# TimD1/vcfdist

Hardware: AMD Instinct MI355X
Metric: supercluster-alignments/sec (higher is better)
Workload: dtype int32; 1 GPU; wgs_synth; superclusters_per_gpu=1000000, span_dist=lognormal(median 20, sigma 1.2) clip [4,10000]

## Files before the change

include/vcfdist_pr.h:

```cpp
#ifndef VCFDIST_PR_H_
#define VCFDIST_PR_H_

#include <stddef.h>
#include <stdint.h>

#ifdef __cplusplus
extern "C" {
#endif

#define VPR_HAPS 4
#define VPR_ALNS 4

#define VPR_PTR_VARIANT 1
#define VPR_PTR_VAR_BEG 2
#define VPR_PTR_VAR_END 4
#define VPR_PTR_INS_LOC 8

#define VPR_TYPE_SUB 1
#define VPR_TYPE_INS 2
#define VPR_TYPE_DEL 3

#define VPR_ERRTYPE_TP 0
#define VPR_ERRTYPE_FP 1
#define VPR_ERRTYPE_FN 2
// ... 42 lines not shown

typedef struct vpr_variants {
    int32_t n_sc;
    int32_t n_ctg;
    const int64_t *ctg_off;
    const uint8_t *ctg_seq;
    const int32_t *sc_ctg;
    const int32_t *sc_beg;
    const int32_t *sc_end;
    const int64_t *var_off[VPR_HAPS];
    const int32_t *var_pos[VPR_HAPS];
    const uint8_t *var_type[VPR_HAPS];
    const float   *var_qual[VPR_HAPS];
    const int64_t *var_ref_off[VPR_HAPS];
    const int32_t *var_ref_len[VPR_HAPS];
    const int64_t *var_alt_off[VPR_HAPS];
    const int32_t *var_alt_len[VPR_HAPS];
    const uint8_t *allele_pool[VPR_HAPS];
} vpr_variants;

typedef struct vpr_config {
    int32_t device;
    float   max_qual;
    double  credit_threshold;
    double  phase_threshold;
    int64_t workspace_bytes;
    int32_t band_mode;
    int32_t flags;
} vpr_config;
#define VPR_CFG_DENSE_S16 1
#define VPR_CFG_TIE_SMALL_LOGS 2
#define VPR_CFG_GUARD_ALLOC 4
#define VPR_CFG_HAP_DEDUP 16
#define VPR_CFG_KEEP_PATHS 8

typedef struct vpr_results {
    int32_t  *aln_dist;
    uint8_t  *aln_end_plane;
    uint8_t  *aln_beg_plane;
    uint32_t *aln_status;
    int32_t  *sc_phase;
    int32_t  *orig_phase_dist;
    int32_t  *swap_phase_dist;
    uint8_t  *errtype[VPR_HAPS][2];
    int32_t  *sync_group[VPR_HAPS][2];
    float    *credit[VPR_HAPS][2];
    int32_t  *ref_ed[VPR_HAPS][2];
    int32_t  *query_ed[VPR_HAPS][2];
    float    *callq[VPR_HAPS][2];
} vpr_results;

typedef struct vpr_timing {
    double ms_total;
    double ms_prep;
    double ms_fwd;
    double ms_bwd;
    double ms_walk;
    double ms_ed;
    int64_t n_fwd_launches;
    int64_t cells_dense;
    int64_t cells_touched;
    int64_t bytes_algorithmic;
    int64_t n_band_retries;
    int64_t n_tie_replays;
    double  ms_tie;
    double  ms_wall;
// ... 114 lines not shown
```

vcfdist_amd/_abi.py:

```python
import ctypes as C

import numpy as np

HAPS = 4
ALNS = 4

PTR_VARIANT, PTR_VAR_BEG, PTR_VAR_END, PTR_INS_LOC = 1, 2, 4, 8
TYPE_SUB, TYPE_INS, TYPE_DEL = 1, 2, 3
ERRTYPE_TP, ERRTYPE_FP, ERRTYPE_FN, ERRTYPE_UN = 0, 1, 2, 5
PHASE_ORIG, PHASE_SWAP, PHASE_NONE = 0, 1, 2
PLANE_QUERY, PLANE_REF = 0, 1

ST_SWAP_TIE = 1
ST_WARN_REF_ED = 2
ST_WARN_QUERY_ED = 4
ST_WARN_EXCEEDS = 8
ST_WARN_ZERO_ED = 16
ST_ERR_NO_PTR = 32
ST_ERR_UNFINISHED = 64
ST_ERR_LIMIT = 128
ST_WARN_MASK = ST_WARN_REF_ED | ST_WARN_QUERY_ED | ST_WARN_EXCEEDS | ST_WARN_ZERO_ED

P_i64 = C.POINTER(C.c_int64)
P_i32 = C.POINTER(C.c_int32)
# ... 18 lines not shown
    _fields_ = [
        ("n_sc", C.c_int32), ("n_ctg", C.c_int32),
        ("ctg_off", P_i64), ("ctg_seq", P_u8),
        ("sc_ctg", P_i32), ("sc_beg", P_i32), ("sc_end", P_i32),
        ("var_off", P_i64 * HAPS), ("var_pos", P_i32 * HAPS), ("var_type", P_u8 * HAPS),
        ("var_qual", P_f32 * HAPS), ("var_ref_off", P_i64 * HAPS), ("var_ref_len", P_i32 * HAPS),
        ("var_alt_off", P_i64 * HAPS), ("var_alt_len", P_i32 * HAPS),
        ("allele_pool", P_u8 * HAPS),
    ]


class VprConfig(C.Structure):
    _fields_ = [
        ("device", C.c_int32), ("max_qual", C.c_float),
        ("credit_threshold", C.c_double), ("phase_threshold", C.c_double),
        ("workspace_bytes", C.c_int64), ("band_mode", C.c_int32), ("flags", C.c_int32),
    ]


class VprResults(C.Structure):
    _fields_ = [
        ("aln_dist", P_i32), ("aln_end_plane", P_u8), ("aln_beg_plane", P_u8), ("aln_status", P_u32),
        ("sc_phase", P_i32), ("orig_phase_dist", P_i32), ("swap_phase_dist", P_i32),
        ("errtype", (P_u8 * 2) * HAPS), ("sync_group", (P_i32 * 2) * HAPS),
        ("credit", (P_f32 * 2) * HAPS), ("ref_ed", (P_i32 * 2) * HAPS),
        ("query_ed", (P_i32 * 2) * HAPS), ("callq", (P_f32 * 2) * HAPS),
    ]


CFG_DENSE_S16 = 1
CFG_TIE_SMALL_LOGS = 2
CFG_GUARD_ALLOC = 4
CFG_KEEP_PATHS = 8
CFG_HAP_DEDUP = 16


class VprTiming(C.Structure):
    _fields_ = [
        ("ms_total", C.c_double), ("ms_prep", C.c_double), ("ms_fwd", C.c_double),
        ("ms_bwd", C.c_double), ("ms_walk", C.c_double), ("ms_ed", C.c_double),
        ("n_fwd_launches", C.c_int64), ("cells_dense", C.c_int64), ("cells_touched", C.c_int64),
        ("bytes_algorithmic", C.c_int64), ("n_band_retries", C.c_int64),
        ("n_tie_replays", C.c_int64), ("ms_tie", C.c_double),
        ("ms_wall", C.c_double), ("ms_wall_phase", C.c_double * 6), ("ms_host_alloc", C.c_double),
        ("ms_host_blocked", C.c_double), ("n_alignments_computed", C.c_int64), ("n_device_allocs", C.c_int64), ("n_device_frees", C.c_int64),
        ("n_host_allocs", C.c_int64), ("n_lane1_seen", C.c_int64), ("n_lane1_finished", C.c_int64), ("n_lane1_waves_dropped", C.c_int64),
    ]


class VprLaunchStat(C.Structure):
    _fields_ = [
        ("kind", C.c_int32), ("threads", C.c_int32), ("cells_per_thread", C.c_int32), ("n_units", C.c_int32),
        ("cells", C.c_int64), ("bytes_algorithmic", C.c_int64), ("ms", C.c_double),
        ("cells_dense", C.c_int64), ("kernel", C.c_char * 32),
    ]


class VprSynthParams(C.Structure):
    _fields_ = [
        ("seed", C.c_uint64), ("n_sc", C.c_int32), ("len_mode", C.c_int32),
        ("len_a", C.c_double), ("len_b", C.c_double),
        ("len_min", C.c_int32), ("len_max", C.c_int32),
        ("p_repeat", C.c_double), ("var_per_base", C.c_double), ("p_snp", C.c_double),
        ("indel_mean", C.c_double), ("p_hom", C.c_double), ("p_keep", C.c_double),
        ("p_drop", C.c_double), ("max_qual", C.c_int32), ("reserved", C.c_int32),
        ("p_sv", C.c_double), ("sv_min", C.c_int32), ("sv_max", C.c_int32),
# ... 462 lines not shown
```

vcfdist_amd/csrc/pr_api.hip:

```cpp
#include <hip/hip_runtime.h>
#include <hip/hip_ext.h>
#include <dlfcn.h>

#include <algorithm>
#include <atomic>
#include <chrono>
#include <cstdarg>
#include <cstdio>
#include <cstdlib>
#include <cstring>
#include <condition_variable>
#include <deque>
#include <functional>
#include <mutex>
#include <string>
#include <thread>
#include <tuple>
#include <unordered_map>
#include <unordered_set>
#include <vector>

#include "../../include/vcfdist_pr.h"
#include "pr_device.h"
#include "pr_plan.h"
// ... 61 lines not shown
}
__global__ void __launch_bounds__(64) k_zl_hdr(BatchOffsets O, const int32_t *__restrict__ order, int n_short, ZlWave *__restrict__ hdr) {
    const int w = blockIdx.x, lane = threadIdx.x;
    const int j = w * 64 + lane;
    int lq = 0, lr = 0, lt = 0;
    if (j < n_short) {
        const int a = order[j];
        const int sc = a >> 2, i = a & 3, qs = i >> 1, ts = 2 + (i & 1);
        lq = int32_t(O.hap_off[qs][sc + 1] - O.hap_off[qs][sc]);
        lt = int32_t(O.hap_off[ts][sc + 1] - O.hap_off[ts][sc]);
        lr = int32_t(O.ref_off[sc + 1] - O.ref_off[sc]);
    }
#pragma unroll
    for (int o = 32; o; o >>= 1) {
        lq = max(lq, __shfl_xor(lq, o)); lr = max(lr, __shfl_xor(lr, o)); lt = max(lt, __shfl_xor(lt, o));
    }
    if (lane == 0) {
        ZlWave W;
        W.in_off = 0; W.log_off = 0; W.mq = lq; W.mr = lr; W.mt = lt; W.pad = 0;
        hdr[w] = W;
    }
}
__global__ void __launch_bounds__(1024) k_zl_scan(ZlWave *__restrict__ hdr, int n_waves, int64_t *__restrict__ totals) {
    __shared__ int64_t s_in[1024], s_log[1024];
    __shared__ int s_len;
    const int tid = threadIdx.x;
    if (tid == 0) s_len = 0;
    const int per = (n_waves + 1023) / 1024;
    const int b = min(n_waves, tid * per), e = min(n_waves, b + per);
    int64_t si = 0, sl = 0;
    int lm = 0;
    for (int k = b; k < e; k++) {
        const ZlWave W = hdr[k];
        si += 64 * (int64_t(W.mq) + W.mr + W.mt); sl += 80 * int64_t(W.mt);
        lm = max(lm, max(W.mq, max(W.mr, W.mt)));
    }
    s_in[tid] = si; s_log[tid] = sl;
    __syncthreads();
    for (int o = 1; o < 1024; o <<= 1) {
        const int64_t ai = tid >= o ? s_in[tid - o] : 0, al = tid >= o ? s_log[tid - o] : 0;
        __syncthreads();
        s_in[tid] += ai; s_log[tid] += al;
        __syncthreads();
    }
    int64_t oi = s_in[tid] - si, ol = s_log[tid] - sl;
    for (int k = b; k < e; k++) {
        ZlWave W = hdr[k];
        W.in_off = oi; W.log_off = ol;
        oi += 64 * (int64_t(W.mq) + W.mr + W.mt); ol += 80 * int64_t(W.mt);
        hdr[k] = W;
    }
    if (lm) atomicMax(&s_len, lm);
    __syncthreads();
    if (tid == 1023) { totals[0] = s_in[1023]; totals[1] = s_log[1023]; totals[2] = s_len; }
}


int class_of(int len) {
    for (int k = 0; k < N_CLASSES; k++)
        if (len <= CLASSES[k].max_len) return k;
    return -1;
}

size_t fwd_lds_bytes(int cls, int Lq, int Lr) {
    const int C = CLASSES[cls].c, NT = CLASSES[cls].nt;
    const size_t PQ = (Lq + C - 1) / C * C, PR = (Lr + C - 1) / C * C;
    return (PQ + PR + 8 + 2 * (NT / 64)) * 4;
}
size_t bwd_lds_bytes(int cls, int Lq, int Lr, bool s16 = false) {
    const int C = CLASSES[cls].c, NT = CLASSES[cls].nt;
    const size_t PQ = (Lq + C - 1) / C * C, PR = (Lr + C - 1) / C * C;
    const size_t FQ = (PQ + 16 + 15) & ~size_t(15), FR = (PR + 16 + 15) & ~size_t(15);
    return (((PQ + PR + 8) * (s16 ? 2 : 4) + 15) & ~size_t(15)) + 2 * (FQ + FR) + 4 * (NT / 64) * 4 + 16;
}
bool s16_ok(const AlnDesc &d) { return d.qv_end - d.qv_beg < 32000; }

bool dense_fits(const AlnDesc &d) {
    const int cls = class_of(std::max(d.Lq, d.Lr));
    if (cls < 0 || cls >= STRIP_ONLY_CLS) return false;
    return fwd_lds_bytes(cls, d.Lq, d.Lr) <= LDS_MAX &&
           (bwd_lds_bytes(cls, d.Lq, d.Lr) <= LDS_MAX || (s16_ok(d) && bwd_lds_bytes(cls, d.Lq, d.Lr, true) <= LDS_MAX));
}
// ... 538 lines not shown
int prep_zero_lane(vpr_handle *h) {
    const Plan &P = h->plan0;
    std::vector<ZlWave> &hdr = h->zl_hdr_host;
    hdr.clear();
    h->zl_wave0.assign(P.chunks.size(), 0);
    int64_t in_words = 0, log_max = 0, in_chunk_max = 0, n_short_max = 0;
    int32_t len_max = 0;
    for (size_t ci = 0; ci < P.chunks.size(); ci++) {
        const Chunk &ch = P.chunks[ci];
        h->zl_wave0[ci] = int64_t(hdr.size());
        const int64_t first = ch.work_off + ch.n_long, n_short = ch.count - ch.n_long;
        const int64_t in_words0 = in_words;
        n_short_max = std::max(n_short_max, n_short);
        const size_t w0 = hdr.size(), nw = size_t((n_short + 63) / 64);
        hdr.resize(w0 + nw);
        par_for(nw * 64, [&](size_t b0, size_t e0, int) {
            for (size_t wv = (b0 + 63) / 64; wv * 64 < e0; wv++) {
                ZlWave W;
                memset(&W, 0, sizeof(W));
                for (int64_t j = int64_t(wv) * 64; j < std::min<int64_t>(n_short, int64_t(wv) * 64 + 64); j++) {
                    int32_t Lq, Lr, Lt;
                    h->descs.lens(size_t(P.work[size_t(first + j)]), Lq, Lr, Lt);
                    W.mq = std::max(W.mq, Lq); W.mr = std::max(W.mr, Lr); W.mt = std::max(W.mt, Lt);
                }
                hdr[w0 + wv] = W;
            }
        });
        int64_t log_cur = 0;
        for (size_t wv = 0; wv < nw; wv++) {
            ZlWave &W = hdr[w0 + wv];
            W.in_off = in_words;
            W.log_off = log_cur;
            in_words += 64 * (int64_t(W.mq) + W.mr + W.mt);
            log_cur += 80 * int64_t(W.mt);
            len_max = std::max(len_max, std::max(W.mq, std::max(W.mr, W.mt)));
        }
        log_max = std::max(log_max, log_cur);
        in_chunk_max = std::max(in_chunk_max, in_words - in_words0);
    }
    if (hdr.empty()) return VPR_OK;
    int rc;
    if ((rc = dev_alloc(h, &h->d_zl_hdr, hdr.size()))) return rc;
    HIPCHK(h, hipMemcpyAsync(h->d_zl_hdr, hdr.data(), hdr.size() * sizeof(ZlWave), hipMemcpyHostToDevice, h->stream));
    return zl_finish(h, hdr.size(), in_words, log_max, in_chunk_max, n_short_max, len_max);
}

int zl_finish(vpr_handle *h, size_t n_waves, int64_t in_words, int64_t log_max, int64_t in_chunk_max, int64_t n_short_max, int32_t len_max) {
    const Plan &P = h->plan0;
    int rc;
    if ((rc = dev_alloc(h, &h->d_zl_in, size_t(in_words)))) return rc;
    if ((rc = dev_alloc(h, &h->d_zl_log, size_t(log_max)))) return rc;
    if (!getenv("VPR_NO_D1")) {
        if (const char *e = getenv("VPR_D1_MAX_ROWS")) h->d1_max_rows = std::max(2, atoi(e));
        const double D1_SHARE = 0.4;
        const int64_t D1_FLOOR = int64_t(4) << 20;
        const int64_t slack = 64 * 5 * int64_t(len_max + 1);
        const int64_t in_all = 2 * in_chunk_max + slack, log_all = 2 * log_max + 160 * int64_t((n_short_max + 63) / 64) + 160 * int64_t(len_max + 1);
        h->d1_in_cap = std::min(in_all, std::max(int64_t(D1_SHARE * double(in_all)), D1_FLOOR + slack));
        h->d1_log_cap = std::min(log_all, std::max(int64_t(D1_SHARE * double(log_all)), D1_FLOOR + slack));
        const int64_t cap_ip = std::min<int64_t>(n_short_max, std::max<int64_t>(4096, (n_short_max / 4 + 3) & ~int64_t(3)));
        h->d1_wave_cap = int32_t((cap_ip + 63) / 64);
        h->d1_fail_cap = int32_t(n_short_max + n_short_max / 8 + 1024);
        h->soft_alloc = true;
        rc = dev_alloc(h, &h->d_d1_hdr, size_t(h->d1_wave_cap));
        if (!rc) rc = dev_alloc(h, &h->d_d1_in, size_t(h->d1_in_cap));
        if (!rc) rc = dev_alloc(h, &h->d_d1_log, size_t(h->d1_log_cap));
        if (!rc) rc = dev_alloc(h, &h->d_d1_fail, size_t(h->d1_fail_cap));
        if (!rc) rc = dev_alloc(h, &h->d_d1_info, 16);
        if (!rc) rc = dev_alloc(h, &h->d_d1_blk, size_t(h->d1_fail_cap / 256 + 8));
        h->soft_alloc = false;
        if (rc) {
            if (h->debug) fprintf(stderr, "[vpr] distance-1 lane level: no room for its blocks (%.2f GB), the level is off for this batch\n",
                                  double(h->d1_in_cap) * 4e-9 + double(h->d1_log_cap) * 16e-9);
            h->d_d1_hdr = nullptr; h->d_d1_in = nullptr; h->d_d1_log = nullptr; h->d_d1_fail = nullptr; h->d_d1_info = nullptr; h->d_d1_blk = nullptr;
            h->err.clear();
            (void)hipGetLastError();
        } else {
            HIPCHK(h, hipMemsetAsync(h->d_d1_info, 0, 64, h->stream));
        }
    }
    for (size_t ci = 0; ci < P.chunks.size(); ci++) {
        const Chunk &ch = P.chunks[ci];
        const int64_t n_short = ch.count - ch.n_long;
        if (n_short <= 0) continue;
        hipLaunchKernelGGL(k_prep_zl, dim3(unsigned((n_short + 63) / 64)), dim3(256), 0, h->stream, h->dB, h->d_descs,
                           P.d_work + ch.work_off + ch.n_long, int(n_short), h->d_zl_hdr + h->zl_wave0[ci], h->d_zl_in);
    }
    HIPCHK(h, hipGetLastError());
    if (h->debug) fprintf(stderr, "[vpr] zero-distance lane level: %zu waves, %.2f GB position words, %.2f GB log\n", n_waves,
                          double(in_words) * 4e-9, double(log_max) * 16e-9);
// ... 561 lines not shown
        void *pf = nullptr, *pc = nullptr, *pl = nullptr, *pt = nullptr;
        { int rc_pin = pin_alloc(h, &pf, n_fail * sizeof(int32_t)); if (rc_pin) return rc_pin; }
        { int rc_pin = pin_alloc(h, &pc, n_slots * sizeof(int32_t)); if (rc_pin) return rc_pin; }
        { int rc_pin = pin_alloc(h, &pl, size_t(h->tie_list_cap) * sizeof(int4)); if (rc_pin) return rc_pin; }
        { int rc_pin = pin_alloc(h, &pt, 32 * sizeof(int32_t)); if (rc_pin) return rc_pin; }
        h->hp_fail = static_cast<int32_t *>(pf);
        h->hp_cnt = static_cast<int32_t *>(pc);
        h->hp_tie_list = static_cast<int4 *>(pl);
        h->hp_tie_cnt = static_cast<int32_t *>(pt);
        h->hp_flag = h->hp_tie_cnt + 8;
        memset(h->hp_cnt, 0, n_slots * sizeof(int32_t));
        memset(h->hp_tie_cnt, 0, 32 * sizeof(int32_t));
    }

    lap("result/aux allocations");
    size_t free_b = 0, total_b = 0;
    HIPCHK(h, hipMemGetInfo(&free_b, &total_b));
    {
        const int64_t fb = books_free(int64_t(free_b), int64_t(total_b));
        if (h->debug && fb != int64_t(free_b)) fprintf(stderr, "[vpr] memory plan: the driver reports %.1f GB free, the books %.1f\n", double(free_b) / 1e9, double(fb) / 1e9);
        free_b = size_t(fb);
    }
    int64_t avail = int64_t(free_b), avail_cache = 0;
    for (const auto &c : h->dev_cache) avail_cache += int64_t(c.bytes);
    avail += avail_cache;
    int64_t scratch_kept = 0;
    for (int k = 0; k < 4; k++) for (int e = 0; e < 2; e++) scratch_kept += h->lad[k].tie_scratch_bytes[e];
    avail += scratch_kept;
    h->mem_reserve = int64_t(double(total_b) * free_share());
    avail = std::max<int64_t>(avail - h->mem_reserve, avail / 2);
    int64_t lane_est = 0;
    if (h->p0.valid && h->cfg.band_mode != 0 && h->cfg.band_mode != 2) {
        const double zl = 1.15 * (double(h->p0.part_in[1]) / 6.0 * 4.0 + 20.0 * double(h->p0.part_rows[1]));
        lane_est = int64_t(zl * (getenv("VPR_NO_D1") ? 1.0 : 1.8)) + 28 * int64_t(h->descs.size());
        avail = std::max<int64_t>(avail - lane_est, avail / 2);
    }
    int64_t budget = h->cfg.workspace_bytes > 0 ? h->cfg.workspace_bytes : int64_t(double(avail) * arena_share());
    if (budget < (8 << 20)) budget = 8 << 20;
    int64_t want = 0;
    {
        const int bm = h->cfg.band_mode;
        const bool q16ok = (bm == 1 || bm == 3);
        std::vector<int64_t> wants(PAR_MAX, 0);
        if (h->p0.valid) wants[0] = h->p0.need128 * 128 + 4096;
        else
        par_for(h->descs.size(), [&](size_t b0, size_t e0, int tid) {
          int64_t want = 0;
          for (size_t k = b0; k < e0; k++) {
            const AlnDesc &d = h->descs[k];
            int64_t flags;
            if (bm != 0 && q16ok && d.Lt < h->long_lt) {
                const int64_t nstr = (int64_t(d.Lt) + 3) / 4;
                flags = nstr * 128 + round_up(nstr * 8, 64);
            } else if (bm != 0) {
                const int W = (q16ok && bm != 2) ? LV_WINDOW[LONG_LV] : 64;
                flags = round_up(round_up(std::min(W, d.Lq), 16) * int64_t(d.Lt), 64) +
                        round_up(round_up(std::min(W, d.Lr), 16) * int64_t(d.Lt), 64) + round_up(8 * int64_t(d.Lt), 64);
            } else {
                flags = round_up(round_up(d.Lq, 32) * int64_t(d.Lt), 64) + round_up(round_up(d.Lr, 32) * int64_t(d.Lt), 64);
            }
            want += flags + round_up(int64_t(d.path_cap) * int64_t(sizeof(PathEnt)) + 128, 128) + 256;
          }
          wants[size_t(tid)] = want;
        });
        for (int64_t w : wants) want += w;
        if (h->cfg.workspace_bytes <= 0) budget = std::min(budget, std::max<int64_t>(want, 256 << 20));
    }
// ... 774 lines not shown
        }
        if ((phases & 2) && !zero) {
        ls.bytes_algorithmic = ls.cells;
        rc = timed(2, ls, ks, band_bwd_name(lv), [&] {
            if (q16)
                hipLaunchKernelGGL(k_bwd_q16, dim3((cnt + 3) / 4), dim3(64), 0, ks, h->dB, h->d_descs, list, cnt,
                                   P.arena, a_i32, h->d_outs, tag, dtag, n_dev);
            else
                hipLaunchKernelGGL(band_bwd_kernel(lv), dim3(cnt), dim3(lv >= LV_C4 ? W : 64), 0,
                                   ks, h->dB, h->d_descs, list, P.arena, a_i32, h->d_outs, tag);
        });
        if (rc) return rc;
        }
        if (!(phases & 4)) return rc;
        const bool wave_walk = !q16 && (long_part || cnt < 2048);
        int64_t walk_rows_sum = 0;
        if (lv == LV_C1 && !h->seq_walk)
            for (int32_t k = 0; k < cnt && walk_rows_sum <= WSEG_MAX_ROWS; k++) walk_rows_sum += plan_desc(h, P, size_t(off) + size_t(k)).Lt;
        const bool seg_walk = lv == LV_C1 && !h->seq_walk && walk_rows_sum <= WSEG_MAX_ROWS;
        const bool row_walk = lv == LV_C1 && (wave_walk || seg_walk);
        vpr_launch_stat ws_;
        memset(&ws_, 0, sizeof(ws_));
        ws_.threads = q16 ? 16 : 64; ws_.n_units = cnt; ws_.cells_per_thread = 2;
        if (q16) {
            if (!zero) rc = timed(3, ws_, ks, "k_walk_q16", [&] {
                hipLaunchKernelGGL(k_walk_q16, dim3((cnt + 3) / 4), dim3(64), 0, ks, h->dB, h->d_descs, list, cnt,
                                   P.arena, a_i32, h->d_outs, a_path, tag, dtag, n_dev);
            });
            if (rc) return rc;
            ws_.cells_per_thread = 3;
            if (zero) ws_.bytes_algorithmic = 20 * zl_rows;
            if (zero) rc = timed(3, ws_, ks, "k_zero_tail", [&] {
                hipLaunchKernelGGL(k_zero_tail, dim3((cnt + 63) / 64), dim3(64), 0, ks, h->dB, h->d_descs, list, cnt, h->d_zl_hdr + zl_wave0,
                                   h->d_zl_in, h->d_zl_log, h->d_outs, a_path, (h->cfg.flags & VPR_CFG_KEEP_PATHS) ? 1 : 0, h->d_secs,
                                   h->d_fp_table, h->d_jobs, h->d_njobs, h->jobs_cap, tag, h->lane_prio_rows);
            });
            else if (cnt <= CREDIT_WAVE_MAX && !n_dev) rc = timed(3, ws_, ks, "k_credit<wave>", [&] {
                hipLaunchKernelGGL(k_credit<true>, dim3(cnt), dim3(64), 0, ks, h->dB, h->d_descs, list, cnt,
                                   h->d_outs, a_path, h->d_secs, h->d_fp_table, h->d_jobs, h->d_njobs,
                                   h->jobs_cap, dtag, tag, n_dev);
            });
            else {
                static const int head_max = [] { const char *e = exp_getenv("VPR_CREDIT_HEAD"); return e ? atoi(e) : 4096; }();
                const int32_t head = (n_dev && h->d_d1_blk && cnt > 2 * head_max) ? head_max : 0;
                if (head > 0) {
                    vpr_launch_stat wh_ = ws_;
                    wh_.n_units = head;
                    rc = timed(3, wh_, ks, "k_credit<wave>", [&] {
                        hipLaunchKernelGGL(k_credit<true>, dim3(head), dim3(64), 0, ks, h->dB, h->d_descs, list, head,
                                           h->d_outs, a_path, h->d_secs, h->d_fp_table, h->d_jobs, h->d_njobs,
                                           h->jobs_cap, dtag, tag, n_dev, 0);
                    });
                    if (rc) return rc;
                }
                rc = timed(3, ws_, ks, "k_credit<lane>", [&] {
                    hipLaunchKernelGGL(k_credit<false>, dim3((cnt - head + 63) / 64), dim3(64), 0, ks, h->dB, h->d_descs,
                                       list, cnt, h->d_outs, a_path, h->d_secs, h->d_fp_table, h->d_jobs,
                                       h->d_njobs, h->jobs_cap, dtag, tag, n_dev, int(head));
                });
            }
        } else if (row_walk) {
            static const int wseg_min_rows = [] { const char *e = exp_getenv("VPR_WSEG_MIN_ROWS"); return e ? atoi(e) : 2048; }();
            int32_t n_seg = cnt;
            if (seg_walk && long_part && wseg_min_rows > 0) {
                n_seg = 0;
                while (n_seg < cnt && plan_desc(h, P, size_t(off) + size_t(n_seg)).Lt >= wseg_min_rows) n_seg++;
            }
// ... 1024 lines not shown
```

vcfdist_amd/csrc/pr_device.h:

```cpp
#ifndef PR_DEVICE_H_
#define PR_DEVICE_H_
#include <hip/hip_runtime.h>
#include <stdint.h>

#define F_INS 1
#define F_DEL 2
#define F_MAT 4
#define F_SUB 8
#define F_SWP 16
#define F_CHOICE_SHIFT 5
#define F_TIE 128
#define F_CHOICE_MASK (0x60u | F_SUB)
__host__ __device__ __forceinline__ uint32_t f_choice_bits(int rank) { return (uint32_t(rank & 3) << F_CHOICE_SHIFT) | (uint32_t(rank >> 2) << 3); }
__host__ __device__ __forceinline__ int f_choice_of(uint32_t f) { return int(((f >> F_CHOICE_SHIFT) & 3u) | ((f >> 1) & 4u)); }
__host__ __device__ __forceinline__ uint32_t f_diag(uint32_t f) { return f & (F_MAT | (F_SUB & ~(f >> 1))); }
__host__ __device__ __forceinline__ uint32_t rank_bits(int rank) { return (uint32_t(rank & 3) << 1) | (uint32_t(rank >> 2) << 4); }
__host__ __device__ __forceinline__ int rank_of(uint32_t bits) { return int(((bits >> 1) & 3u) | ((bits >> 2) & 4u)); }
#define F_SWP_KEY_MASK (F_SWP | F_CHOICE_MASK)
__host__ __device__ __forceinline__ uint32_t f_swp_key(int rank) { return F_SWP | f_choice_bits(rank); }
#define SWAP_SOURCES_MAX 8
#define F_KEEP 0xe0

#define PV 1
#define PB 2
// ... 154 lines not shown
        d.band_w = 16;
        d.pitch[0] = d.pitch[1] = 16;
        m0 = nstr * 128; m1 = 0;
        bl = round_up64(nstr * 8, 128);
    } else {
        d.band_w = W;
        d.pitch[0] = int32_t(round_up64(W < d.Lq ? W : d.Lq, 16));
        d.pitch[1] = int32_t(round_up64(W < d.Lr ? W : d.Lr, 16));
        m0 = round_up64(int64_t(d.pitch[0]) * d.Lt, 128); m1 = round_up64(int64_t(d.pitch[1]) * d.Lt, 128);
        bl = round_up64(int64_t(2) * d.Lt * 4, 128);
    }
    const int64_t pb = round_up64(int64_t(d.path_cap) * int64_t(sizeof(PathEnt)) + 128, 128);
    d.band_pad = lv_tag(dl) | tag_or;
    d.mat_off[0] = used;
    d.mat_off[1] = used + m0;
    d.blo_off = (used + m0 + m1) / 4;
    d.path_off = (used + m0 + m1 + bl) / int64_t(sizeof(PathEnt));
    return m0 + m1 + bl + pb + 128;
}

__host__ __device__ inline int alias_source(int b, int i) {
    const int q = i >> 1, t = i & 1;
    const int qs = (b & 1) ? 0 : q, ts = (b & 2) ? 0 : t;
    const int src = qs * 2 + ts;
    return src == i ? -1 : src;
}

struct ZlWave {
    int64_t in_off;
    int64_t log_off;
    int32_t mq, mr, mt;
    int32_t pad;
};
struct TieJob;

#endif
```

vcfdist_amd/csrc/pr_zl.hip:

```cpp
#ifndef PR_ZL_HIP_
#define PR_ZL_HIP_
#include <type_traits>


#define ZW_PTR(w) (int((w) & 0xffffu) - 1)
#define ZW_BASE(w) (((w) >> 16) & 0x7fu)
#define ZW_PV (1u << 23)
#define ZW_PB (1u << 24)
#define ZW_PE (1u << 25)
#define ZW_INS (1u << 26)
#define ZW_TP (1u << 27)
__device__ __forceinline__ bool zw_fwd_allow(uint32_t w) { return !(w & ZW_PV) || (w & ZW_PE); }
__device__ __forceinline__ bool zw_bwd_allow(uint32_t w) { return !(w & ZW_PV) || (w & ZW_PB); }

#define ZE_ALIVE 1u
#define ZE_HASMAT 2u
#define ZE_HASSWP 4u
#define ZE_PSLOT_SHIFT 3
#define ZE_TP 32u
#define ZE_BWD 64u

#define ZL_MAXLEN 65000
#define ZL_CLEAN_REJECT (-1)

// ... 47 lines not shown
                    if (arr == 0 && x > 0 && ((p != wk[o - 1].x + 1) || (f & PB))) v |= ZW_TP;
                    (void)Lr;
                }
                tile[lane][l] = v;
            }
            __syncthreads();
            const int rows = min(64, mlen - x0);
            for (int r = sub; r < rows; r += 4) out[int64_t(x0 + r) * 64 + lane] = tile[r][lane];
            __syncthreads();
        }
        out += int64_t(mlen) * 64;
    }
}

typedef __attribute__((ext_vector_type(4))) unsigned int zl_u4;
typedef __attribute__((ext_vector_type(2))) unsigned int zl_u2;
#define ZL_OOB 0xfffffff0u

__global__ void __launch_bounds__(64, 6) k_zero_lane(const AlnDesc *__restrict__ descs, const int32_t *__restrict__ list, int n_list,
                                                  const ZlWave *__restrict__ hdr, const uint32_t *__restrict__ zin,
                                                  uint4 *__restrict__ zlog, AlnOut *__restrict__ outs, PathEnt *__restrict__ paths,
                                                  int keep_paths, int d1_max_rows, int prio_rows) {
    const int w = blockIdx.x, lane = threadIdx.x;
    const ZlWave H = hdr[w];
    if (H.mt >= prio_rows) __builtin_amdgcn_s_setprio(2);
    const int wi = w * 64 + lane;
    const int a_ = wi < n_list ? list[wi] : -1;
    const bool live = a_ >= 0;
    const int a = max(a_, 0);
    const AlnDesc *dp = descs + a;
    const int Lq = live ? dp->Lq : 1, Lr = live ? dp->Lr : 1, Lt = live ? dp->Lt : 0;
    const int L[2] = {Lq, Lr};
    const auto rin = __builtin_amdgcn_make_buffer_rsrc(const_cast<uint32_t *>(zin + H.in_off), 0, 256 * (H.mq + H.mr + H.mt), 0x00020000);
    const auto rlog = __builtin_amdgcn_make_buffer_rsrc(zlog + H.log_off, 0, 1280 * H.mt, 0x00020000);
    const uint32_t lane4 = uint32_t(lane) << 2, lane8 = uint32_t(lane) << 3;
    const uint32_t pos0[2] = {0u, uint32_t(H.mq) << 8}, post = uint32_t(H.mq + H.mr) << 8;
    const uint32_t logP0 = uint32_t(H.mt) << 9;
    auto in_at = [&](uint32_t off) -> uint32_t { return __builtin_amdgcn_raw_buffer_load_b32(rin, off, 0, 0); };
    bool ok = live && Lq < ZL_MAXLEN && Lr < ZL_MAXLEN && Lt < ZL_MAXLEN && Lt >= 2;
    const int rows = ok ? Lt : 0;
    int tmax = rows;
#pragma unroll
    for (int o = 32; o; o >>= 1) tmax = max(tmax, __shfl_xor(tmax, o));
    if (tmax == 0) {
        if (live) { outs[a].dist_q = D_INF; outs[a].dist_r = D_INF; outs[a].exit_min = 0; }
        return;
    }

    int qri[2][4];
    uint32_t pw[2][4];
#pragma unroll
    for (int p = 0; p < 2; p++) {
#pragma unroll
        for (int s = 0; s < 4; s++) { qri[p][s] = -1; pw[p][s] = 0; }
    }
    uint32_t tw0 = in_at(ok ? post + lane4 : ZL_OOB);
    if (ok) {
        qri[0][0] = 0; pw[0][0] = in_at(pos0[0] + lane4);
        qri[1][0] = 0; pw[1][0] = in_at(pos0[1] + lane4);
        zl_u2 e0;
        e0.x = ZE_ALIVE | ZE_HASMAT | ((pw[0][0] & ZW_TP) ? ZE_TP : 0u) | (zw_bwd_allow(pw[0][0]) ? ZE_BWD : 0u);
        e0.y = ZE_ALIVE | ZE_HASMAT | (zw_bwd_allow(pw[1][0]) ? ZE_BWD : 0u);
        __builtin_amdgcn_raw_buffer_store_b64(e0, rlog, lane8, 0, 0);
    }
    uint32_t pf_mw[2][2] = {{0, 0}, {0, 0}}, pf_sw[2][2] = {{0, 0}, {0, 0}};
    bool have_pf = false;
    auto fwd_row = [&](auto Sc, int t, bool act, uint32_t tw1) -> bool {
        constexpr int S = decltype(Sc)::value;
        const bool t_allow = zw_fwd_allow(tw0);
        uint32_t mw[2][S], sw[2][S];
        int sz[2][S];
        const bool use_pf = S == 2 && have_pf;
#pragma unroll
        for (int p = 0; p < 2; p++) {
#pragma unroll
            for (int s = 0; s < S; s++) {
                const bool alive = act && qri[p][s] >= 0;
                const int c = qri[p][s] + 1;
                const int z = ZW_PTR(pw[p][s]) + 1;
                const bool sok = alive && t_allow && zw_fwd_allow(pw[p][s]) && z < L[1 - p];
                sz[p][s] = sok ? z : -1;
                if (use_pf) {
                    mw[p][s] = (alive && c < L[p]) ? pf_mw[p][s & 1] : 0u;
                    sw[p][s] = sok ? pf_sw[p][s & 1] : 0u;
                } else {
                    mw[p][s] = in_at((alive && c < L[p]) ? pos0[p] + (uint32_t(c) << 8) + lane4 : ZL_OOB);
                    sw[p][s] = in_at(sok ? pos0[1 - p] + (uint32_t(z) << 8) + lane4 : ZL_OOB);
                }
            }
        }
        const uint32_t Tb = ZW_BASE(tw1);
        int nq[2][S];
        uint32_t nw[2][S], ne[2][S];
#pragma unroll
        for (int p = 0; p < 2; p++) {
#pragma unroll
// ... 1 lines not shown
                const bool hit = act && qri[p][s] >= 0 && ZW_BASE(mw[p][s]) == Tb;
                nq[p][s] = hit ? qri[p][s] + 1 : -1;
                nw[p][s] = mw[p][s];
                ne[p][s] = hit ? ZE_HASMAT : 0u;
            }
        }
        bool bad = false, full = false;
#pragma unroll
        for (int p = 0; p < 2; p++) {
            const int o = 1 - p;
#pragma unroll
            for (int s = 0; s < S; s++) {
                const bool hit = sz[p][s] >= 0 && ZW_BASE(sw[p][s]) == Tb;
                if (!__any(hit)) continue;
                const int z = sz[p][s];
                int at = -1;
#pragma unroll
                for (int k = S - 1; k >= 0; k--) at = (nq[o][k] < 0) ? k : at;
#pragma unroll
                for (int k = 0; k < S; k++) at = (nq[o][k] == z) ? k : at;
                full = full || (hit && at < 0);
#pragma unroll
                for (int k = 0; k < S; k++) {
                    const bool here = hit && at == k;
                    bad = bad || (here && (ne[o][k] & ZE_HASSWP));
                    nq[o][k] = here ? z : nq[o][k];
                    nw[o][k] = here ? sw[p][s] : nw[o][k];
                    ne[o][k] = here ? (ne[o][k] | ZE_HASSWP | (uint32_t(s) << ZE_PSLOT_SHIFT)) : ne[o][k];
                }
            }
        }
        if (S < 4 && __any(full)) return false;
        ok = ok && !bad && !full;
        if (S == 2) {
#pragma unroll
            for (int p = 0; p < 2; p++) {
#pragma unroll
                for (int s = 0; s < 2; s++) {
                    const bool alive = act && ok && nq[p][s] >= 0;
                    const int c = nq[p][s] + 1;
                    const int z = ZW_PTR(nw[p][s]) + 1;
                    pf_mw[p][s] = in_at((alive && c < L[p]) ? pos0[p] + (uint32_t(c) << 8) + lane4 : ZL_OOB);
                    pf_sw[p][s] = in_at((alive && zw_fwd_allow(nw[p][s]) && z < L[1 - p]) ? pos0[1 - p] + (uint32_t(z) << 8) + lane4 : ZL_OOB);
                }
            }
        }
        have_pf = S == 2;
        {
            zl_u2 ev;
            uint32_t wq = 0, wr_ = 0;
#pragma unroll
            for (int sl = 0; sl < S; sl++) {
                wq |= (nq[0][sl] < 0 ? 0u : (ZE_ALIVE | ne[0][sl] | ((nw[0][sl] & ZW_TP) ? ZE_TP : 0u) | (zw_bwd_allow(nw[0][sl]) ? ZE_BWD : 0u))) << (8 * sl);
                wr_ |= (nq[1][sl] < 0 ? 0u : (ZE_ALIVE | ne[1][sl] | (zw_bwd_allow(nw[1][sl]) ? ZE_BWD : 0u))) << (8 * sl);
            }
            ev.x = wq; ev.y = wr_;
            __builtin_amdgcn_raw_buffer_store_b64(ev, rlog, (act && ok) ? (uint32_t(t + 1) << 9) + lane8 : ZL_OOB, 0, 0);
        }
#pragma unroll
        for (int p = 0; p < 2; p++) {
#pragma unroll
            for (int s = 0; s < S; s++) { qri[p][s] = act ? nq[p][s] : qri[p][s]; pw[p][s] = act ? nw[p][s] : pw[p][s]; }
        }
        tw0 = act ? tw1 : tw0;
        return true;
    };
    for (int t = 0; t + 1 < tmax; t++) {
        const bool act = ok && t + 1 < rows;
        const uint32_t tw1 = in_at(act ? post + (uint32_t(t + 1) << 8) + lane4 : ZL_OOB);
        bool upper = false;
#pragma unroll
        for (int p = 0; p < 2; p++) upper = upper || (act && (qri[p][2] >= 0 || qri[p][3] >= 0));
        if (__any(upper) || !fwd_row(std::integral_constant<int, 2>{}, t, act, tw1))
            (void)fwd_row(std::integral_constant<int, 4>{}, t, act, tw1);
    }
    int endq = -1, endr = -1;
#pragma unroll
    for (int s = 0; s < 4; s++) {
        if (qri[0][s] == Lq - 1) endq = s;
        if (qri[1][s] == Lr - 1) endr = s;
    }
    const bool clean = ok && Lt <= d1_max_rows;
    ok = ok && (endq >= 0 || endr >= 0);
    if (live) {
        AlnOut &o = outs[a];
        o.dist_q = (ok && endq >= 0) ? 0 : D_INF;
        o.dist_r = (ok && endr >= 0) ? 0 : D_INF;
        o.exit_min = ok ? D_INF : (clean ? ZL_CLEAN_REJECT : 0);
    }
    if (!__any(ok)) return;

    const int nrow = ok ? Lt : 0;
    int sc[2][4];
#pragma unroll
    for (int p = 0; p < 2; p++) {
#pragma unroll
        for (int s = 0; s < 4; s++) sc[p][s] = -1;
    }
    int bmax = nrow;
#pragma unroll
    for (int o = 32; o; o >>= 1) bmax = max(bmax, __shfl_xor(bmax, o));
    auto log_row = [&](int t, bool on) -> zl_u2 {
        return __builtin_amdgcn_raw_buffer_load_b64(rlog, on ? (uint32_t(t) << 9) + lane8 : ZL_OOB, 0, 0);
    };
    zl_u2 cur = zl_u2{0, 0};
    auto bwd_row = [&](auto Sc, int t, bool act, zl_u2 pre) {
        constexpr int S = decltype(Sc)::value;
        int best[2][S];
        uint32_t pp[2][S];
#pragma unroll
        for (int p = 0; p < 2; p++) {
#pragma unroll
            for (int s = 0; s < S; s++) { best[p][s] = -1; pp[p][s] = 0; }
        }
#pragma unroll
        for (int p = 0; p < 2; p++) {
            const int o = 1 - p;
#pragma unroll
            for (int s = 0; s < S; s++) {
                const bool on = act && sc[p][s] >= 0;
                const uint32_t e = ((p ? cur.y : cur.x) >> (8 * s)) & 0xffu;
                const int tp = (e & ZE_TP) ? 1 : 0;
                {
                    const bool m = on && (e & ZE_HASMAT);
                    const int v = sc[p][s] + tp;
// ... 76 lines not shown
        e.a = (v.x & 0xffffu) | (((v.x >> 16) & 1u) << 31);
        e.b = uint32_t(i) | (((v.x >> 17) & 1u) << 31) | (((v.x >> 18) & 3u) << 28);
        e.qref = int(v.y & 0xffffu) - 1;
        e.tref = int(v.y >> 16) - 1;
        return e;
    }
};

__global__ void __launch_bounds__(64) k_zero_tail(DevBatch B, const AlnDesc *__restrict__ descs, const int32_t *__restrict__ list, int n_list,
                                                  const ZlWave *__restrict__ hdr, const uint32_t *__restrict__ zin,
                                                  uint4 *__restrict__ zlog, AlnOut *__restrict__ outs, PathEnt *__restrict__ paths,
                                                  int keep_paths, Section *__restrict__ secs, int32_t *const *__restrict__ fp_group,
                                                  EdJob *__restrict__ jobs, int32_t *__restrict__ n_jobs, int32_t jobs_cap, int tag,
                                                  int prio_rows) {
    const int w = blockIdx.x, lane = threadIdx.x;
    const ZlWave H = hdr[w];
    if (H.mt >= prio_rows) __builtin_amdgcn_s_setprio(2);
    const int wi = w * 64 + lane;
    const int a_ = wi < n_list ? list[wi] : -1;
    const bool live = a_ >= 0;
    const int a = max(a_, 0);
    const AlnDesc d = descs[a];
    AlnOut &O = outs[a];
    const bool ok = live && d.band_pad == tag && O.band_ok == tag;
    const int nrow = ok ? d.Lt : 0;
    int bmax = nrow;
#pragma unroll
    for (int o = 32; o; o >>= 1) bmax = max(bmax, __shfl_xor(bmax, o));
    if (bmax == 0) return;
    uint32_t status = ok ? O.status : 0u;
    bool wok = ok;
    {
        const auto rin = __builtin_amdgcn_make_buffer_rsrc(const_cast<uint32_t *>(zin + H.in_off), 0, 256 * (H.mq + H.mr + H.mt), 0x00020000);
        const auto rlog = __builtin_amdgcn_make_buffer_rsrc(zlog + H.log_off, 0, 1280 * H.mt, 0x00020000);
        const uint32_t lane4 = uint32_t(lane) << 2, lane8 = uint32_t(lane) << 3;
        const uint32_t pos0[2] = {0u, uint32_t(H.mq) << 8}, post = uint32_t(H.mq + H.mr) << 8;
        const uint32_t logP0 = uint32_t(H.mt) << 9, logS0 = logP0 + (uint32_t(H.mt) << 8);
        auto in_at = [&](uint32_t off) -> uint32_t { return __builtin_amdgcn_raw_buffer_load_b32(rin, off, 0, 0); };
        const int beg_plane = ok ? O.beg_plane : 0;
        PathEnt *path = paths + d.path_off;
        int hi = beg_plane, slot = 0, mv_in = 0, x = 0;
        uint32_t wstatus = 0;
        for (int t = 0; t < bmax; t++) {
            const bool act = wok && t < nrow;
            const uint32_t ppw = __builtin_amdgcn_raw_buffer_load_b32(rlog, (act && t + 1 < nrow) ? logP0 + (uint32_t(t) << 8) + lane4 : ZL_OOB, 0, 0);
            const uint32_t tw = in_at(act ? post + (uint32_t(t) << 8) + lane4 : ZL_OOB);
            const uint32_t cw = in_at(act ? pos0[hi] + (uint32_t(x) << 8) + lane4 : ZL_OOB);
            const int trv = ZW_PTR(tw), qref = hi ? x : ZW_PTR(cw);
            uint32_t sync = 1;
            if (mv_in) {
                const bool in_t = (tw & ZW_PV) && !(tw & ZW_PB);
                const bool in_q = hi == 0 && (cw & ZW_PV) && !(cw & ZW_PB);
                sync = (!in_t && !in_q && !((tw | cw) & ZW_INS) && trv == qref) ? 1u : 0u;
            }
            const uint32_t eqb = (ZW_BASE(cw) == ZW_BASE(tw) ? 1u : 0u) | ((hi || !(cw & ZW_PV)) ? 2u : 0u);
            zl_u2 st;
            st.x = uint32_t(x) | (uint32_t(hi) << 16) | (sync << 17) | (eqb << 18);
            st.y = uint32_t(qref + 1) | (uint32_t(trv + 1) << 16);
            __builtin_amdgcn_raw_buffer_store_b64(st, rlog, act ? logS0 + (uint32_t(t) << 9) + lane8 : ZL_OOB, 0, 0);
            if ((keep_paths & 1) && act) {
                uint4 pe;
                pe.x = uint32_t(x) | (uint32_t(hi) << 31);
                pe.y = uint32_t(t) | (sync << 31);
                pe.z = uint32_t(qref);
                pe.w = uint32_t(trv);
                *reinterpret_cast<uint4 *>(path + t) = pe;
            }
            if (act && t + 1 < nrow) {
                const uint32_t nb = (ppw >> (4 * ((hi << 2) | slot))) & 15u;
                if (hi == 1 && (nb & 2u)) { hi = 0; slot = int(nb >> 2); x = ZW_PTR(cw) + 1; }
                else if (nb & 1u) { x = x + 1; }
                else if (hi == 0 && (nb & 2u)) { hi = 1; slot = int(nb >> 2); x = ZW_PTR(cw) + 1; }
                else { wstatus |= VPR_ST_ERR_NO_PTR; wok = false; }
                mv_in = 1;
            }
        }
        if (ok) {
            O.path_len = wok ? nrow : 0;
            if (!wok) O.n_sec = 0;
            if (wstatus) atomicOr(&O.status, wstatus);
        }
        status |= wstatus;
    }
    asm volatile("s_waitcnt vmcnt(0)" ::: "memory");
    if (!ok || (status & (VPR_ST_ERR_NO_PTR | VPR_ST_ERR_LIMIT))) return;
    ZlFetch f{reinterpret_cast<const uint2 *>(zlog + H.log_off + 48 * int64_t(H.mt)) + lane, -1, make_uint2(0, 0)};
    credit_walk<false, ZlFetch, true>(B, d, O, a, nullptr, int64_t(wok ? nrow : 0), 0u, secs, fp_group, jobs, n_jobs, jobs_cap, true, f);
}

#endif
```

Baseline: 202.7 million supercluster-alignments/s.

## Log per-row slot words in forward pass and prefetch walk rows ahead

The forward zero-lane kernel now stores a 128-bit record per row holding the input words of the two low slots for each plane, so the backward walk no longer needs a data-dependent load of the current input word in most cases. The walk loop is software-pipelined four rows deep, issuing the pointer, target and slot-record loads for row t+4 while row t is processed. A fallback dependent load is kept for slots >= 2 or when the new WALK_DEP_LOADS flag is set. The cost is a larger log region per row (144 units instead of 80), extra stores in the forward pass, and a larger workspace estimate.

```diff
diff --git a/include/vcfdist_pr.h b/include/vcfdist_pr.h
--- a/include/vcfdist_pr.h
+++ b/include/vcfdist_pr.h
@@ -98,6 +98,7 @@
 #define VPR_CFG_TIE_SMALL_LOGS 2
 #define VPR_CFG_GUARD_ALLOC 4
 #define VPR_CFG_HAP_DEDUP 16
+#define VPR_CFG_WALK_DEP_LOADS 32
 #define VPR_CFG_KEEP_PATHS 8
 
 typedef struct vpr_results {
diff --git a/vcfdist_amd/_abi.py b/vcfdist_amd/_abi.py
--- a/vcfdist_amd/_abi.py
+++ b/vcfdist_amd/_abi.py
@@ -74,6 +74,7 @@
 CFG_TIE_SMALL_LOGS = 2
 CFG_GUARD_ALLOC = 4
 CFG_KEEP_PATHS = 8
+CFG_WALK_DEP_LOADS = 32
 CFG_HAP_DEDUP = 16
 
 
diff --git a/vcfdist_amd/csrc/pr_api.hip b/vcfdist_amd/csrc/pr_api.hip
--- a/vcfdist_amd/csrc/pr_api.hip
+++ b/vcfdist_amd/csrc/pr_api.hip
@@ -117,7 +117,7 @@
     int lm = 0;
     for (int k = b; k < e; k++) {
         const ZlWave W = hdr[k];
-        si += 64 * (int64_t(W.mq) + W.mr + W.mt); sl += 80 * int64_t(W.mt);
+        si += 64 * (int64_t(W.mq) + W.mr + W.mt); sl += ZL_LOG_UNITS * int64_t(W.mt);
         lm = max(lm, max(W.mq, max(W.mr, W.mt)));
     }
     s_in[tid] = si; s_log[tid] = sl;
@@ -132,7 +132,7 @@
     for (int k = b; k < e; k++) {
         ZlWave W = hdr[k];
         W.in_off = oi; W.log_off = ol;
-        oi += 64 * (int64_t(W.mq) + W.mr + W.mt); ol += 80 * int64_t(W.mt);
+        oi += 64 * (int64_t(W.mq) + W.mr + W.mt); ol += ZL_LOG_UNITS * int64_t(W.mt);
         hdr[k] = W;
     }
     if (lm) atomicMax(&s_len, lm);
@@ -737,7 +737,7 @@
             W.in_off = in_words;
             W.log_off = log_cur;
             in_words += 64 * (int64_t(W.mq) + W.mr + W.mt);
-            log_cur += 80 * int64_t(W.mt);
+            log_cur += ZL_LOG_UNITS * int64_t(W.mt);
             len_max = std::max(len_max, std::max(W.mq, std::max(W.mr, W.mt)));
         }
         log_max = std::max(log_max, log_cur);
@@ -760,7 +760,8 @@
         const double D1_SHARE = 0.4;
         const int64_t D1_FLOOR = int64_t(4) << 20;
         const int64_t slack = 64 * 5 * int64_t(len_max + 1);
-        const int64_t in_all = 2 * in_chunk_max + slack, log_all = 2 * log_max + 160 * int64_t((n_short_max + 63) / 64) + 160 * int64_t(len_max + 1);
+        const int64_t log_max_d1 = log_max / ZL_LOG_UNITS * ZL_LOG_UNITS_D1;
+        const int64_t in_all = 2 * in_chunk_max + slack, log_all = 2 * log_max_d1 + 160 * int64_t((n_short_max + 63) / 64) + 160 * int64_t(len_max + 1);
         h->d1_in_cap = std::min(in_all, std::max(int64_t(D1_SHARE * double(in_all)), D1_FLOOR + slack));
         h->d1_log_cap = std::min(log_all, std::max(int64_t(D1_SHARE * double(log_all)), D1_FLOOR + slack));
         const int64_t cap_ip = std::min<int64_t>(n_short_max, std::max<int64_t>(4096, (n_short_max / 4 + 3) & ~int64_t(3)));
@@ -1388,7 +1389,8 @@
     int64_t lane_est = 0;
     if (h->p0.valid && h->cfg.band_mode != 0 && h->cfg.band_mode != 2) {
         const double zl = 1.15 * (double(h->p0.part_in[1]) / 6.0 * 4.0 + 20.0 * double(h->p0.part_rows[1]));
-        lane_est = int64_t(zl * (getenv("VPR_NO_D1") ? 1.0 : 1.8)) + 28 * int64_t(h->descs.size());
+        const double zl_slots = 1.15 * 16.0 * double(h->p0.part_rows[1]);
+        lane_est = int64_t(zl * (getenv("VPR_NO_D1") ? 1.0 : 1.8) + zl_slots) + 28 * int64_t(h->descs.size());
         avail = std::max<int64_t>(avail - lane_est, avail / 2);
     }
     int64_t budget = h->cfg.workspace_bytes > 0 ? h->cfg.workspace_bytes : int64_t(double(avail) * arena_share());
@@ -2229,7 +2231,8 @@
             if (zero) ws_.bytes_algorithmic = 20 * zl_rows;
             if (zero) rc = timed(3, ws_, ks, "k_zero_tail", [&] {
                 hipLaunchKernelGGL(k_zero_tail, dim3((cnt + 63) / 64), dim3(64), 0, ks, h->dB, h->d_descs, list, cnt, h->d_zl_hdr + zl_wave0,
-                                   h->d_zl_in, h->d_zl_log, h->d_outs, a_path, (h->cfg.flags & VPR_CFG_KEEP_PATHS) ? 1 : 0, h->d_secs,
+                                   h->d_zl_in, h->d_zl_log, h->d_outs, a_path,
+                                   ((h->cfg.flags & VPR_CFG_KEEP_PATHS) ? 1 : 0) | ((h->cfg.flags & VPR_CFG_WALK_DEP_LOADS) ? 2 : 0), h->d_secs,
                                    h->d_fp_table, h->d_jobs, h->d_njobs, h->jobs_cap, tag, h->lane_prio_rows);
             });
             else if (cnt <= CREDIT_WAVE_MAX && !n_dev) rc = timed(3, ws_, ks, "k_credit<wave>", [&] {
diff --git a/vcfdist_amd/csrc/pr_device.h b/vcfdist_amd/csrc/pr_device.h
--- a/vcfdist_amd/csrc/pr_device.h
+++ b/vcfdist_amd/csrc/pr_device.h
@@ -210,6 +210,8 @@
     int32_t mq, mr, mt;
     int32_t pad;
 };
+#define ZL_LOG_UNITS 144
+#define ZL_LOG_UNITS_D1 80
 struct TieJob;
 
 #endif
diff --git a/vcfdist_amd/csrc/pr_zl.hip b/vcfdist_amd/csrc/pr_zl.hip
--- a/vcfdist_amd/csrc/pr_zl.hip
+++ b/vcfdist_amd/csrc/pr_zl.hip
@@ -103,10 +103,10 @@
     const int Lq = live ? dp->Lq : 1, Lr = live ? dp->Lr : 1, Lt = live ? dp->Lt : 0;
     const int L[2] = {Lq, Lr};
     const auto rin = __builtin_amdgcn_make_buffer_rsrc(const_cast<uint32_t *>(zin + H.in_off), 0, 256 * (H.mq + H.mr + H.mt), 0x00020000);
-    const auto rlog = __builtin_amdgcn_make_buffer_rsrc(zlog + H.log_off, 0, 1280 * H.mt, 0x00020000);
-    const uint32_t lane4 = uint32_t(lane) << 2, lane8 = uint32_t(lane) << 3;
+    const auto rlog = __builtin_amdgcn_make_buffer_rsrc(zlog + H.log_off, 0, 16 * ZL_LOG_UNITS * H.mt, 0x00020000);
+    const uint32_t lane4 = uint32_t(lane) << 2, lane8 = uint32_t(lane) << 3, lane16 = uint32_t(lane) << 4;
     const uint32_t pos0[2] = {0u, uint32_t(H.mq) << 8}, post = uint32_t(H.mq + H.mr) << 8;
-    const uint32_t logP0 = uint32_t(H.mt) << 9;
+    const uint32_t logP0 = uint32_t(H.mt) << 9, logW0 = uint32_t(H.mt) * 1280u;
     auto in_at = [&](uint32_t off) -> uint32_t { return __builtin_amdgcn_raw_buffer_load_b32(rin, off, 0, 0); };
     bool ok = live && Lq < ZL_MAXLEN && Lr < ZL_MAXLEN && Lt < ZL_MAXLEN && Lt >= 2;
     const int rows = ok ? Lt : 0;
@@ -133,6 +133,7 @@
         e0.x = ZE_ALIVE | ZE_HASMAT | ((pw[0][0] & ZW_TP) ? ZE_TP : 0u) | (zw_bwd_allow(pw[0][0]) ? ZE_BWD : 0u);
         e0.y = ZE_ALIVE | ZE_HASMAT | (zw_bwd_allow(pw[1][0]) ? ZE_BWD : 0u);
         __builtin_amdgcn_raw_buffer_store_b64(e0, rlog, lane8, 0, 0);
+        __builtin_amdgcn_raw_buffer_store_b128(zl_u4{pw[0][0], 0u, pw[1][0], 0u}, rlog, logW0 + lane16, 0, 0);
     }
     uint32_t pf_mw[2][2] = {{0, 0}, {0, 0}}, pf_sw[2][2] = {{0, 0}, {0, 0}};
     bool have_pf = false;
@@ -200,6 +201,8 @@
         }
         if (S < 4 && __any(full)) return false;
         ok = ok && !bad && !full;
+        __builtin_amdgcn_raw_buffer_store_b128(zl_u4{nq[0][0] < 0 ? 0u : nw[0][0], nq[0][1] < 0 ? 0u : nw[0][1], nq[1][0] < 0 ? 0u : nw[1][0], nq[1][1] < 0 ? 0u : nw[1][1]}, rlog,
+                                               (act && ok) ? logW0 + (uint32_t(t + 1) << 10) + lane16 : ZL_OOB, 0, 0);
         if (S == 2) {
 #pragma unroll
             for (int p = 0; p < 2; p++) {
@@ -248,7 +251,7 @@
         if (qri[0][s] == Lq - 1) endq = s;
         if (qri[1][s] == Lr - 1) endr = s;
     }
-    const bool clean = ok && Lt <= d1_max_rows;
+    const bool clean = ok && rows <= d1_max_rows;
     ok = ok && (endq >= 0 || endr >= 0);
     if (live) {
         AlnOut &o = outs[a];
@@ -258,7 +261,7 @@
     }
     if (!__any(ok)) return;
 
-    const int nrow = ok ? Lt : 0;
+    const int nrow = ok ? rows : 0;
     int sc[2][4];
 #pragma unroll
     for (int p = 0; p < 2; p++) {
@@ -401,20 +404,33 @@
     bool wok = ok;
     {
         const auto rin = __builtin_amdgcn_make_buffer_rsrc(const_cast<uint32_t *>(zin + H.in_off), 0, 256 * (H.mq + H.mr + H.mt), 0x00020000);
-        const auto rlog = __builtin_amdgcn_make_buffer_rsrc(zlog + H.log_off, 0, 1280 * H.mt, 0x00020000);
-        const uint32_t lane4 = uint32_t(lane) << 2, lane8 = uint32_t(lane) << 3;
+        const auto rlog = __builtin_amdgcn_make_buffer_rsrc(zlog + H.log_off, 0, 16 * ZL_LOG_UNITS * H.mt, 0x00020000);
+        const uint32_t lane4 = uint32_t(lane) << 2, lane8 = uint32_t(lane) << 3, lane16 = uint32_t(lane) << 4;
         const uint32_t pos0[2] = {0u, uint32_t(H.mq) << 8}, post = uint32_t(H.mq + H.mr) << 8;
-        const uint32_t logP0 = uint32_t(H.mt) << 9, logS0 = logP0 + (uint32_t(H.mt) << 8);
+        const uint32_t logP0 = uint32_t(H.mt) << 9, logS0 = logP0 + (uint32_t(H.mt) << 8), logW0 = logS0 + (uint32_t(H.mt) << 9);
         auto in_at = [&](uint32_t off) -> uint32_t { return __builtin_amdgcn_raw_buffer_load_b32(rin, off, 0, 0); };
         const int beg_plane = ok ? O.beg_plane : 0;
         PathEnt *path = paths + d.path_off;
+        const bool dep_all = (keep_paths & 2) != 0;
         int hi = beg_plane, slot = 0, mv_in = 0, x = 0;
         uint32_t wstatus = 0;
-        for (int t = 0; t < bmax; t++) {
+        struct WRow { uint32_t ppw, tw; zl_u4 sl; };
+        auto row_req = [&](int r, WRow &R) {
+            const bool on = ok && r < nrow;
+            R.ppw = __builtin_amdgcn_raw_buffer_load_b32(rlog, (on && r + 1 < nrow) ? logP0 + (uint32_t(r) << 8) + lane4 : ZL_OOB, 0, 0);
+            R.tw = in_at(on ? post + (uint32_t(r) << 8) + lane4 : ZL_OOB);
+            R.sl = __builtin_amdgcn_raw_buffer_load_b128(rlog, on ? logW0 + (uint32_t(r) << 10) + lane16 : ZL_OOB, 0, 0);
+        };
+        auto walk_step = [&](int t, WRow &R) {
             const bool act = wok && t < nrow;
-            const uint32_t ppw = __builtin_amdgcn_raw_buffer_load_b32(rlog, (act && t + 1 < nrow) ? logP0 + (uint32_t(t) << 8) + lane4 : ZL_OOB, 0, 0);
-            const uint32_t tw = in_at(act ? post + (uint32_t(t) << 8) + lane4 : ZL_OOB);
-            const uint32_t cw = in_at(act ? pos0[hi] + (uint32_t(x) << 8) + lane4 : ZL_OOB);
+            const uint32_t ppw = R.ppw, tw = act ? R.tw : 0u;
+            const uint32_t ms = 0u - uint32_t(slot & 1), mh = 0u - uint32_t(hi);
+            const uint32_t cq = (R.sl.x & ~ms) | (R.sl.y & ms), cr = (R.sl.z & ~ms) | (R.sl.w & ms);
+            uint32_t cw = act ? ((cq & ~mh) | (cr & mh)) : 0u;
+            if (dep_all || __any(act && slot >= 2)) {
+                cw = in_at(act ? pos0[hi] + (uint32_t(x) << 8) + lane4 : ZL_OOB);
+                __builtin_amdgcn_s_waitcnt(0x0f70);
+            }
             const int trv = ZW_PTR(tw), qref = hi ? x : ZW_PTR(cw);
             uint32_t sync = 1;
             if (mv_in) {
@@ -443,6 +459,15 @@
                 else { wstatus |= VPR_ST_ERR_NO_PTR; wok = false; }
                 mv_in = 1;
             }
+            row_req(t + 4, R);
+        };
+        WRow rA, rB, rC, rD;
+        row_req(0, rA); row_req(1, rB); row_req(2, rC); row_req(3, rD);
+        for (int t = 0; t < bmax; t += 4) {
+            walk_step(t, rA);
+            walk_step(t + 1, rB);
+            walk_step(t + 2, rC);
+            walk_step(t + 3, rD);
         }
         if (ok) {
             O.path_len = wok ? nrow : 0;
```

New measurement: 194.3 million supercluster-alignments/s. 4.2% lower.
